# xuyongzhi/Automatic-As-built-Reconstruction

Measured on AMD Instinct MI355X. Metric: scenes/sec (fwd+bwd), higher is better.
Workload: dtype f32

## Files before the change

automatic-as-built-reconstruction_amd/csrc/common.h:

```cpp
#pragma once
#include <hip/hip_runtime.h>
#include <stdint.h>
#include <stdio.h>
#include <atomic>
#include "../../include/aabr_hip.h"
#include "conv_tiles.h"

namespace aabr {

void set_error(const char *fmt, ...);

typedef float f32x4 __attribute__((ext_vector_type(4)));
typedef unsigned int u32x4 __attribute__((ext_vector_type(4)));
typedef __bf16 bf16x8 __attribute__((ext_vector_type(8)));

#define AABR_KNOB_LIST(X)                                                                                            \
  X(CONV_WLDS) X(CONV_SMALL) X(CONV_NBW) X(CONV_WPB) X(WIDE_ROWS) X(CONV_WIDE) X(WIDE_NBUF) X(CONV_WIDE_BF16)         \
  X(VOXEL_MEAN) X(WIDE_NCB) X(BN_SMALL) X(WIDE_PRIO) X(PLAN_SIDE_BATCH) X(PLAN_SIDE_PRIO) X(SMALL_WPB) X(SMALL_MAX)   \
  X(WIDE_SPLIT) X(SPLIT_TARGET) X(SPLIT_NBUF) X(SPLIT_MIN_ITEMS) X(CONV_NARROW) X(DW_FULL) X(DW_FULL_MIN) X(DW_FULL_WGS) X(DW_VEC) X(SPLIT_ROWS) X(GEOM_JOBS)      \
  X(CONV_SINGLE) X(SINGLE_ROWS) X(SINGLE_CHUNK) X(SINGLE_BWD_STATS) X(PLAN_TAIL)
#define AABR_KNOB_ENUM(n) K_##n,
enum Knob { AABR_KNOB_LIST(AABR_KNOB_ENUM) K_COUNT };
#undef AABR_KNOB_ENUM
int knob(Knob k);

#define AABR_CHECK_ARG_AS(fn, cond, msg)                            \
  do {                                                              \
    if (!(cond)) { aabr::set_error("%s: %s", fn, msg); return AABR_EINVAL; } \
  } while (0)
#define AABR_CHECK_ARG(cond, msg) AABR_CHECK_ARG_AS(__func__, cond, msg)

#define AABR_CHECK_LAUNCH()                                                   \
  do {                                                                        \
    hipError_t e__ = hipGetLastError();                                       \
    if (e__ != hipSuccess) {                                                  \
      aabr::set_error("%s: HIP error %s", __func__, hipGetErrorString(e__));  \
      return AABR_ELAUNCH;                                                    \
    }                                                                         \
  } while (0)

#define AABR_CHECK_HIP(call)                                                  \
  do {                                                                        \
    hipError_t e__ = (call);                                                  \
    if (e__ != hipSuccess) {                                                  \
      aabr::set_error("%s: HIP error %s", __func__, hipGetErrorString(e__));  \
      return AABR_ELAUNCH;                                                    \
    }                                                                         \
  } while (0)

struct DynLdsOnce {
  std::atomic<uint64_t> done{0};
};
inline hipError_t dyn_lds_once(DynLdsOnce &o, const void *kernel, int bytes) {
  int dev = 0;
  hipError_t e = hipGetDevice(&dev);
  if (e != hipSuccess) return e;
  const uint64_t bit = dev < 64 ? 1ull << dev : 0ull;
  if (o.done.load(std::memory_order_acquire) & bit) return hipSuccess;
  e = hipFuncSetAttribute(kernel, hipFuncAttributeMaxDynamicSharedMemorySize, bytes);
  if (e == hipSuccess) o.done.fetch_or(bit, std::memory_order_release);
  return e;
}

constexpr uint64_t kEmptyKey = 0xFFFFFFFFFFFFFFFFull;
constexpr int kMaxCoord = 65534;

__host__ __device__ inline uint64_t pack_key(int b, int x, int y, int z) {
  return ((uint64_t)(uint32_t)(b & 0xffff) << 48) | ((uint64_t)(uint32_t)((x + 1) & 0xffff) << 32) |
         ((uint64_t)(uint32_t)((y + 1) & 0xffff) << 16) | (uint64_t)(uint32_t)((z + 1) & 0xffff);
}
__host__ __device__ inline bool coord_in_range(int v) { return v >= -1 && v <= kMaxCoord; }

__host__ __device__ inline uint64_t mix64(uint64_t k) {
  k ^= k >> 33; k *= 0xff51afd7ed558ccdull; k ^= k >> 33;
  k *= 0xc4ceb9fe1a85ec53ull; k ^= k >> 33;
  return k;
}

struct __align__(16) GridEnt {
  unsigned long long key;
  uint32_t first;
  int32_t val;
};
static_assert(sizeof(GridEnt) == 16, "GridEnt is 16 bytes");

constexpr uint32_t kGridBlock = 4096;
__device__ inline uint64_t grid_next(uint64_t h, uint64_t mask, uint32_t t) {
  const uint64_t bm = mask < (uint64_t)(kGridBlock - 1) ? mask : (uint64_t)(kGridBlock - 1);
  return t < bm ? ((h & ~bm) | ((h + 1) & bm)) : (((t == bm ? (h | bm) : h) + 1) & mask);
}

__device__ inline int grid_find(const GridEnt *__restrict__ g, uint64_t mask, uint64_t key) {
  uint64_t h = mix64(key) & mask;
  for (uint32_t t = 0;; ++t) {
    const uint4 e = *reinterpret_cast<const uint4 *>(g + h);
    const uint64_t k = (uint64_t)e.x | ((uint64_t)e.y << 32);
    if (k == key) return (int)e.w;
    if (k == kEmptyKey) return -1;
    h = grid_next(h, mask, t);
  }
}

__device__ inline uint32_t grid_insert(GridEnt *g, uint64_t mask, uint64_t key) {
  uint64_t h = mix64(key) & mask;
  for (uint32_t t = 0;; ++t) {
    unsigned long long prev = atomicCAS(&g[h].key, (unsigned long long)kEmptyKey, (unsigned long long)key);
    if (prev == kEmptyKey || prev == key) return (uint32_t)h;
    h = grid_next(h, mask, t);
  }
}

constexpr int kStreamJobsMax = 48;
struct StreamJob {
  const int32_t *table;
  const int32_t *counts;
  int32_t *words;
  int64_t V;
  int32_t vol, T;
};
struct StreamJobs {
  StreamJob j[kStreamJobsMax];
  uint32_t first[kStreamJobsMax + 1];
  int n;
};
__device__ inline int stream_job_of(const StreamJobs &js, unsigned b) {
  int j = 0;
  while (j + 1 < js.n && b >= js.first[j + 1]) ++j;
  return j;
}
int launch_wide_blocks_jobs(const StreamJob *jobs, int n, hipStream_t st);
int launch_tile_blocks_jobs(const StreamJob *jobs, int n, hipStream_t st);
int launch_offset_pairs_jobs(const StreamJob *jobs, int n, hipStream_t st);
constexpr int kSampleJobsMax = 32;
struct SampleJob {
  const int32_t *sc, *meta;
  int32_t *out;
  int64_t V_max;
  int32_t max_samples;
};
int launch_sample_offsets_jobs(const SampleJob *jobs, int n, hipStream_t st);

inline bool is_pow2(int64_t v) { return v > 0 && (v & (v - 1)) == 0; }

}
```

automatic-as-built-reconstruction_amd/csrc/conv_wide.hip:

```cpp
#include "common.h"
#include "conv_wide_tiles.h"
#include <stdlib.h>

namespace aabr {


extern thread_local const char *g_last_variant;

constexpr int kNB = 4;

__global__ __launch_bounds__(256) void k_build_tileT(const StreamJobs js) {
  const int job = stream_job_of(js, blockIdx.x);
  const int32_t *__restrict__ table = js.j[job].table;
  int32_t *__restrict__ words = js.j[job].words;
  const int64_t V = js.j[job].V;
  const int vol = js.j[job].vol, T = js.j[job].T;
  const int kT = T;
  const int NWV = (T + 63) / 64;
  __shared__ int s_cnt[4][kMaxVol];
  __shared__ int s_base[kMaxVol + 1];
  __shared__ int s_tot[kMaxVol];
  __shared__ int s_first[kMaxVol];
  const int wave = threadIdx.x >> 6, lane = threadIdx.x & 63;
  const int64_t ntiles = (V + T - 1) / T, tile = blockIdx.x - js.first[job];
  const int maxb = (T / 16) * vol;
  int32_t *pre = words + tile * (vol + 1);
  int32_t *ent = words + ntiles * (vol + 1) + tile * (int64_t)maxb * 16;
  const int64_t row = tile * kT + threadIdx.x;
  const bool valid = (int)threadIdx.x < T && row < V;
  for (int k = 0; k < vol; ++k) {
    const int t = valid ? table[(int64_t)k * V + row] : -1;
    const unsigned long long m = __ballot(t >= 0);
    if (lane == 0) s_cnt[wave][k] = __popcll(m);
  }
  __syncthreads();
  if (threadIdx.x == 0) {
    int b = 0;
    for (int k = 0; k < vol; ++k) {
      int tot = 0;
      for (int w = 0; w < NWV; ++w) tot += s_cnt[w][k];
      s_tot[k] = tot;
      s_base[k] = b;
      b += (tot + 15) >> 4;
    }
    s_base[vol] = b;
  }
  __syncthreads();
  if ((int)threadIdx.x <= vol) pre[threadIdx.x] = s_base[threadIdx.x];
  for (int k = 0; k < vol; ++k) {
    const int t = valid ? table[(int64_t)k * V + row] : -1;
    const unsigned long long m = __ballot(t >= 0);
    if (t >= 0) {
      int rank = __popcll(m & ((1ull << lane) - 1ull));
      for (int w = 0; w < wave; ++w) rank += s_cnt[w][k];
      const int e = (t << 8) | (int)threadIdx.x;
      ent[s_base[k] * 16 + rank] = e;
      if (rank == 0) s_first[k] = e;
    }
  }
  __syncthreads();
  for (int k = 0; k < vol; ++k) {
    const int tot = s_tot[k];
    if (tot == 0) continue;
    const int pad = ((tot + 15) & ~15) - tot;
    if ((int)threadIdx.x < pad) ent[s_base[k] * 16 + tot + threadIdx.x] = s_first[k] | (int)0x80000000;
  }
}

__device__ inline float bcf_(unsigned int v) { return __builtin_bit_cast(float, v); }


typedef __bf16 bf16x8w __attribute__((ext_vector_type(8)));
typedef __bf16 bf16x4w __attribute__((ext_vector_type(4)));
typedef unsigned int u32x2 __attribute__((ext_vector_type(2)));

struct BnBwdStats {
  const float *x, *mean, *invstd, *weight, *bias;
  float leak;
  const float *out;
};

template <int KG, int DBG, int NBUF, bool BF = false, int NCB = 1, int NSET = 2>
__global__ __launch_bounds__(256, NBUF == 2 ? 2 : 3) void k_conv_cs(const float *__restrict__ in, int ci, int64_t in_bytes,
                                                    float *__restrict__ out, int co, int64_t V_out,
                                                    const int32_t *__restrict__ words, int64_t words_bytes, int vol,
                                                    int wflip, const float *__restrict__ Wp, int64_t wp_bytes,
                                                    const float *__restrict__ bias, int kT2,
                                                    const float *__restrict__ res, double *__restrict__ stats,
                                                    BnBwdStats bn) {
  constexpr int NW = 4;
  constexpr int NT = 64 * NW;
  constexpr int LPR = NT / 32;
  constexpr int RG = KG * 8;
  constexpr int RF = KG * 32;
  constexpr int SWZ = (RG >= 16 && (RG & 15) == 0) ? 15 : 7;
  constexpr int STAGE = 2 * 16 * RF;
  constexpr bool BFM = BF;
  constexpr int NP = 1;
  constexpr int NGL = KG * 8 / LPR;
  extern __shared__ __align__(16) float smem[];
  float *Ct = smem;
  constexpr int WS = 16 * NW * NCB;
  float *St = smem + (kT2 + 1) * WS;
  const int wave = __builtin_amdgcn_readfirstlane(threadIdx.x >> 6), lane = threadIdx.x & 63;
  const int g = lane >> 4, c16 = lane & 15;
  const int pr = wave * (64 / LPR) + lane / LPR, seg = lane % LPR;
  const int nkc = BFM ? ci >> 6 : ci >> 5, nnb = co >> 4;
  const int nparts = (wflip >> 8) & 0xff;
  int64_t tile;
  int nb0, part = 0;
  {
    const unsigned ny = gridDim.y, total = gridDim.x * ny;
    const unsigned lin = blockIdx.y * gridDim.x + blockIdx.x;
    const unsigned per = total >> 3, rem = total & 7u, x = lin & 7u;
    const unsigned wi = x * per + (x < rem ? x : rem) + (lin >> 3);
    tile = wi / ny;
    unsigned sp = wi % ny;
    if (nparts > 1) { part = (int)(sp % (unsigned)nparts); sp /= (unsigned)nparts; }
    nb0 = (int)sp * (NW * NCB);
  }
  const int k_lo = nparts > 1 ? part * vol / nparts : 0;
  const int kend = nparts > 1 ? (part + 1) * vol / nparts : vol;
  const int64_t row0 = tile * kT2;
  const int64_t ntiles = (V_out + kT2 - 1) / kT2;
  const int maxb = (kT2 / 16) * vol;
  const int vpre = lane <= vol ? words[tile * (vol + 1) + lane] : 0;
  {
    f32x4 z = {0.f, 0.f, 0.f, 0.f};
    f32x4 *c4 = reinterpret_cast<f32x4 *>(Ct);
    for (int i = threadIdx.x; i < (kT2 + 1) * WS / 4; i += NT) c4[i] = z;
  }
  const __amdgpu_buffer_rsrc_t rin =
      __builtin_amdgcn_make_buffer_rsrc(const_cast<float *>(in), 0, (int)in_bytes, 0x00020000);
  const __amdgpu_buffer_rsrc_t rwords =
      __builtin_amdgcn_make_buffer_rsrc(const_cast<int32_t *>(words), 0, (int)words_bytes, 0x00020000);
  const __amdgpu_buffer_rsrc_t rw =
      __builtin_amdgcn_make_buffer_rsrc(const_cast<float *>(Wp), 0, (int)wp_bytes, 0x00020000);
  const unsigned ebase = (unsigned)((ntiles * (vol + 1) + tile * (int64_t)maxb * 16) * 4);
  const unsigned rowbytes = (unsigned)ci * (BF ? 2u : 4u);
  const unsigned lane32 = (unsigned)lane * 32u;
  auto pre_of = [&](int k) { return __builtin_amdgcn_readlane(vpre, k); };
  auto next_offset = [&](int k) {
    ++k;
    while (k < kend && pre_of(k + 1) == pre_of(k)) ++k;
    return k;
  };
  struct WReg { u32x4 w0[NP][NCB][KG], w1[NP][NCB][KG]; };
  struct GReg { u32x4 v[NGL]; };
  struct Ent { int eg, ea, eb, hb; };
  const int ngroups = (nkc + KG - 1) / KG;
  const int nblk_all = pre_of(vol);
  auto load_w = [&](WReg &w, int k, int kg) {
    const int kW = (wflip & 1) ? vol - 1 - k : k;
#pragma unroll
    for (int cb = 0; cb < NCB; ++cb)
#pragma unroll
      for (int c = 0; c < KG; ++c) {
        const int kc = kg * KG + c;
        if (BFM) {
          const unsigned so = (unsigned)((((int64_t)kW * (2 * nkc) + 2 * kc) * nnb + nb0 + wave * NCB + cb) * 1024);
#pragma unroll
          for (int pl = 0; pl < NP; ++pl) {
            const unsigned po = so + (unsigned)pl * (unsigned)(wp_bytes / NP);
            w.w0[pl][cb][c] = __builtin_amdgcn_raw_buffer_load_b128(rw, (unsigned)lane * 16u, po, 0);
            w.w1[pl][cb][c] = __builtin_amdgcn_raw_buffer_load_b128(rw, (unsigned)lane * 16u, po + (unsigned)nnb * 1024u, 0);
          }
        } else {
          const unsigned so = (unsigned)((((int64_t)kW * nkc + kc) * nnb + nb0 + wave * NCB + cb) * 2048);
          w.w0[0][cb][c] = __builtin_amdgcn_raw_buffer_load_b128(rw, lane32, so, 0);
          w.w1[0][cb][c] = __builtin_amdgcn_raw_buffer_load_b128(rw, lane32 + 16u, so, 0);
        }
      }
  };
  auto load_ent = [&](int bb, int kk) {
    Ent e;
    const bool hasB = bb + 1 < pre_of(kk + 1);
    const unsigned bA = (unsigned)bb * 64u, bB = (unsigned)(hasB ? bb + 1 : bb) * 64u;
    e.ea = (int)__builtin_amdgcn_raw_buffer_load_b32(rwords, (unsigned)c16 * 4u, ebase + bA, 0);
    e.eb = (int)__builtin_amdgcn_raw_buffer_load_b32(rwords, (unsigned)c16 * 4u, ebase + bB, 0);
    e.eg = (int)__builtin_amdgcn_raw_buffer_load_b32(rwords, (unsigned)(pr & 15) * 4u, ebase + (pr < 16 ? bA : bB), 0);
    if (!hasB) e.eb |= (int)0x80000000;
    e.hb = hasB ? 1 : 0;
    return e;
  };
  auto gather = [&](GReg &q, int eg, int kg) {
    const unsigned va = (((unsigned)eg & 0x7fffffffu) >> 8) * rowbytes + (unsigned)seg * 16u;
#pragma unroll
    for (int i = 0; i < NGL; ++i) {
      const unsigned so = (unsigned)(kg * NGL + i) * (unsigned)(LPR * 16);
      if (DBG & 2) q.v[i] = (u32x4){(unsigned)eg, 0u, 0u, 0u};
      else q.v[i] = __builtin_amdgcn_raw_buffer_load_b128(rin, va, so, 0);
    }
  };
  auto stage_store = [&](const GReg &q, int buf) {
    float *rowp = St + (NBUF == 2 ? buf : 0) * (NP * STAGE) + pr * RF;
#pragma unroll
    for (int i = 0; i < NGL; ++i)
      *reinterpret_cast<u32x4 *>(rowp + (((seg + LPR * i) ^ (pr & SWZ)) << 2)) = q.v[i];
  };
  auto accumulate2 = [&](int ea, const f32x4 (&accA)[NCB], int eb, const f32x4 (&accB)[NCB]) {
    const int ra = ea >= 0 ? (ea & 255) : kT2, rb = eb >= 0 ? (eb & 255) : kT2;
#pragma unroll
    for (int cb = 0; cb < NCB; ++cb) {
      f32x4 *da = reinterpret_cast<f32x4 *>(Ct + ra * WS + ((((wave * NCB + cb) * 4 + g) ^ (ra & 15)) << 2));
      f32x4 *db = reinterpret_cast<f32x4 *>(Ct + rb * WS + ((((wave * NCB + cb) * 4 + g) ^ (rb & 15)) << 2));
      const f32x4 va = *da, vb = *db;
      *da = va + accA[cb];
      *db = vb + accB[cb];
    }
  };
  struct Pos { int b, k; };
  auto adv = [&](Pos q) {
    if (q.k >= kend) return q;
    const int kend = pre_of(q.k + 1);
    q.b += 2;
    if (q.b >= kend) { q.b = kend; q.k = next_offset(q.k); }
    return q;
  };
  auto wg_barrier = [&]() {
    asm volatile("s_waitcnt lgkmcnt(0)\n\ts_barrier" ::: "memory");
  };
  int par = 0;
  long long dbg_t[5] = {0, 0, 0, 0, 0};
  for (int kg = 0; kg < ngroups; ++kg) {
    Pos pp[NSET + 2];
    pp[0].k = next_offset(k_lo - 1);
    if (pp[0].k >= kend) break;
    pp[0].b = pre_of(pp[0].k);
#pragma unroll
    for (int i = 1; i < NSET + 2; ++i) pp[i] = adv(pp[i - 1]);
    auto ent_of = [&](const Pos &q) { const bool v = q.k < kend; return load_ent(v ? q.b : pp[0].b, v ? q.k : pp[0].k); };
    Ent ee[NSET + 2];
#pragma unroll
    for (int i = 0; i <= NSET; ++i) ee[i] = ent_of(pp[i]);
    ee[NSET + 1] = ee[0];
    GReg gq[NSET];
    gather(gq[0], ee[0].eg, kg);
    __syncthreads();
    par = 0;
    int gs = 0;
    stage_store(gq[0], par);
#pragma unroll
    for (int i = 1; i < NSET; ++i) gather(gq[i], ee[i].eg, kg);
    __syncthreads();
    auto step = [&](const WReg &w, GReg &g_issue, GReg &g_store) __attribute__((always_inline)) {
      long long t0 = 0, t1 = 0, t2 = 0, t3 = 0, t4 = 0;
      if (DBG & 4) t0 = __builtin_amdgcn_s_memtime();
      gather(g_issue, ee[NSET].eg, kg);
      ee[NSET + 1] = ent_of(pp[NSET + 1]);
      const Ent e0 = ee[0];
      __builtin_amdgcn_sched_barrier(0);
      if (DBG & 4) { t1 = __builtin_amdgcn_s_memtime(); __builtin_amdgcn_sched_barrier(0); }

      {
        const float *sa = St + (NBUF == 2 ? par : 0) * STAGE + c16 * RF;
        const float *sb = sa + 16 * RF;
        f32x4 accA[NCB], accB[NCB];
#pragma unroll
        for (int cb = 0; cb < NCB; ++cb) { accA[cb] = (f32x4){0.f, 0.f, 0.f, 0.f}; accB[cb] = accA[cb]; }
        if (wflip & 2) __builtin_amdgcn_s_setprio(3);
        {
        u32x4 a0[KG], a1[KG], b0[KG], b1[KG];
#pragma unroll
        for (int c = 0; c < KG; ++c) {
          const int q0 = ((c * 8 + (BF ? g : g * 2)) ^ (c16 & SWZ)) << 2,
                    q1 = ((c * 8 + (BF ? 4 + g : g * 2 + 1)) ^ (c16 & SWZ)) << 2;
          a0[c] = *reinterpret_cast<const u32x4 *>(sa + q0);
          b0[c] = *reinterpret_cast<const u32x4 *>(sb + q0);
          a1[c] = *reinterpret_cast<const u32x4 *>(sa + q1);
          b1[c] = *reinterpret_cast<const u32x4 *>(sb + q1);
        }
        if (DBG & 1) {
#pragma unroll
          for (int c = 0; c < KG; ++c) {
            accA[0][0] += bcf_(a0[c][0]) + bcf_(a1[c][0]) + bcf_(w.w0[0][0][c][0]) + bcf_(w.w1[0][0][c][0]);
            accB[0][0] += bcf_(b0[c][0]) + bcf_(b1[c][0]);
          }
        } else if (BF) {
#pragma unroll
          for (int cb = 0; cb < NCB; ++cb)
#pragma unroll
            for (int c = 0; c < KG; ++c) {
              accA[cb] = __builtin_amdgcn_mfma_f32_16x16x32_bf16(__builtin_bit_cast(bf16x8w, w.w0[0][cb][c]),
                                                                 __builtin_bit_cast(bf16x8w, a0[c]), accA[cb], 0, 0, 0);
              accA[cb] = __builtin_amdgcn_mfma_f32_16x16x32_bf16(__builtin_bit_cast(bf16x8w, w.w1[0][cb][c]),
                                                                 __builtin_bit_cast(bf16x8w, a1[c]), accA[cb], 0, 0, 0);
            }
          if (e0.hb) {
#pragma unroll
            for (int cb = 0; cb < NCB; ++cb)
#pragma unroll
              for (int c = 0; c < KG; ++c) {
                accB[cb] = __builtin_amdgcn_mfma_f32_16x16x32_bf16(__builtin_bit_cast(bf16x8w, w.w0[0][cb][c]),
                                                                   __builtin_bit_cast(bf16x8w, b0[c]), accB[cb], 0, 0, 0);
                accB[cb] = __builtin_amdgcn_mfma_f32_16x16x32_bf16(__builtin_bit_cast(bf16x8w, w.w1[0][cb][c]),
                                                                   __builtin_bit_cast(bf16x8w, b1[c]), accB[cb], 0, 0, 0);
              }
          }
        } else {
#pragma unroll
          for (int cb = 0; cb < NCB; ++cb)
#pragma unroll
            for (int c = 0; c < KG; ++c) {
#pragma unroll
              for (int t = 0; t < 4; ++t)
                accA[cb] = __builtin_amdgcn_mfma_f32_16x16x4f32(bcf_(w.w0[0][cb][c][t]), bcf_(a0[c][t]), accA[cb], 0, 0, 0);
#pragma unroll
              for (int t = 0; t < 4; ++t)
                accA[cb] = __builtin_amdgcn_mfma_f32_16x16x4f32(bcf_(w.w1[0][cb][c][t]), bcf_(a1[c][t]), accA[cb], 0, 0, 0);
            }
          if (e0.hb) {
#pragma unroll
            for (int cb = 0; cb < NCB; ++cb)
#pragma unroll
              for (int c = 0; c < KG; ++c) {
#pragma unroll
                for (int t = 0; t < 4; ++t)
                  accB[cb] = __builtin_amdgcn_mfma_f32_16x16x4f32(bcf_(w.w0[0][cb][c][t]), bcf_(b0[c][t]), accB[cb], 0, 0, 0);
#pragma unroll
                for (int t = 0; t < 4; ++t)
                  accB[cb] = __builtin_amdgcn_mfma_f32_16x16x4f32(bcf_(w.w1[0][cb][c][t]), bcf_(b1[c][t]), accB[cb], 0, 0, 0);
              }
          }
        }
        }
        if (DBG & 4) { __builtin_amdgcn_sched_barrier(0); asm volatile("s_nop 0" ::"v"(accA[0]), "v"(accB[0])); t2 = __builtin_amdgcn_s_memtime(); __builtin_amdgcn_sched_barrier(0); }
        if (wflip & 2) __builtin_amdgcn_s_setprio(0);
        {
          accumulate2(e0.ea, accA, e0.eb, accB);
        }
      }
      {
        if (NBUF == 1) wg_barrier();
        if (pp[1].k < kend) stage_store(g_store, par ^ 1);
      }
      if (DBG & 4) { asm volatile("s_waitcnt lgkmcnt(0)" ::: "memory"); t3 = __builtin_amdgcn_s_memtime(); }
      wg_barrier();
      if (DBG & 4) {
        t4 = __builtin_amdgcn_s_memtime();
        dbg_t[0] += t1 - t0; dbg_t[1] += t2 - t1; dbg_t[2] += t3 - t2; dbg_t[3] += t4 - t3; dbg_t[4] += 1;
      }
      par ^= 1;
#pragma unroll
      for (int i = 0; i < NSET + 1; ++i) { pp[i] = pp[i + 1]; ee[i] = ee[i + 1]; }
      pp[NSET + 1] = adv(pp[NSET + 1]);
    };
    auto step2 = [&](const WReg &w) __attribute__((always_inline)) {
      if (NSET == 2) {
        if (gs == 0) step(w, gq[0], gq[1]);
        else step(w, gq[1], gq[0]);
      } else {
        if (gs == 0) step(w, gq[0], gq[1 % NSET]);
        else if (gs == 1) step(w, gq[1 % NSET], gq[2 % NSET]);
        else if (gs == 2) step(w, gq[2 % NSET], gq[3 % NSET]);
        else step(w, gq[3 % NSET], gq[0]);
      }
      gs = gs + 1 == NSET ? 0 : gs + 1;
    };
    WReg wA;
    int k = pp[0].k;
    load_w(wA, k, kg);
    WReg wB;
    for (;;) {
      int kn = next_offset(k);
      if (kn < kend) load_w(wB, kn, kg);
      while (pp[0].k == k) step2(wA);
      if (kn >= kend) break;
      k = kn;
      kn = next_offset(k);
      if (kn < kend) load_w(wA, kn, kg);
      while (pp[0].k == k) step2(wB);
      if (kn >= kend) break;
      k = kn;
    }
  }
  if (DBG & 4) {
    if (lane == 0) {
      long long *d = reinterpret_cast<long long *>(const_cast<float *>(bias)) +
                     (((int64_t)blockIdx.y * gridDim.x + blockIdx.x) * 4 + wave) * 5;
      for (int q = 0; q < 5; ++q) d[q] = dbg_t[q];
    }
    bias = nullptr;
  }
  __syncthreads();
  const int nrows = (int)((V_out - row0) < kT2 ? (V_out - row0) : kT2);
  constexpr int QW = 4 * NW * NCB;
  if (nparts > 1) {
    float *po = out + (int64_t)part * V_out * co;
    for (int i = threadIdx.x; i < nrows * QW; i += NT) {
      const int r = i / QW, q = i % QW;
      *reinterpret_cast<f32x4 *>(po + (row0 + r) * co + nb0 * 16 + q * 4) =
          *reinterpret_cast<const f32x4 *>(Ct + r * WS + ((q ^ (r & 15)) << 2));
    }
    return;
  }
  double sa[4] = {0.0, 0.0, 0.0, 0.0}, sb[4] = {0.0, 0.0, 0.0, 0.0};
  float bmu[4] = {0.f, 0.f, 0.f, 0.f}, bwc[4] = {0.f, 0.f, 0.f, 0.f}, bbc[4] = {0.f, 0.f, 0.f, 0.f};
  if (stats && bn.x) {
    const int p0 = nb0 * 16 + (threadIdx.x % QW) * 4;
#pragma unroll
    for (int j = 0; j < 4; ++j) {
      bmu[j] = bn.mean[p0 + j];
      if (!BF) {
        bwc[j] = bn.invstd[p0 + j] * (bn.weight ? bn.weight[p0 + j] : 1.0f);
        bbc[j] = -bmu[j] * bwc[j] + (bn.bias ? bn.bias[p0 + j] : 0.0f);
      }
    }
  }
#pragma unroll 4
  for (int i = threadIdx.x; i < nrows * QW; i += NT) {
    const int r = i / QW, q = i % QW;
    f32x4 v = *reinterpret_cast<const f32x4 *>(Ct + r * WS + ((q ^ (r & 15)) << 2));
    if (bias) {
      const float *bb = bias + nb0 * 16 + q * 4;
      v[0] += bb[0]; v[1] += bb[1]; v[2] += bb[2]; v[3] += bb[3];
    }
    if (res) {
      if (BF) {
        const bf16x4w rr = *reinterpret_cast<const bf16x4w *>(reinterpret_cast<const __bf16 *>(res) + (row0 + r) * co +
                                                              nb0 * 16 + q * 4);
#pragma unroll
        for (int j = 0; j < 4; ++j) v[j] = (float)(__bf16)v[j] + (float)rr[j];
      } else {
        const f32x4 rr = *reinterpret_cast<const f32x4 *>(res + (row0 + r) * co + nb0 * 16 + q * 4);
        v[0] += rr[0]; v[1] += rr[1]; v[2] += rr[2]; v[3] += rr[3];
      }
    }
    if (BF) {
      bf16x4w o = {(__bf16)v[0], (__bf16)v[1], (__bf16)v[2], (__bf16)v[3]};
      *reinterpret_cast<bf16x4w *>(reinterpret_cast<__bf16 *>(out) + (row0 + r) * co + nb0 * 16 + q * 4) = o;
      if (stats) { v[0] = (float)o[0]; v[1] = (float)o[1]; v[2] = (float)o[2]; v[3] = (float)o[3]; }
    } else {
      *reinterpret_cast<f32x4 *>(out + (row0 + r) * co + nb0 * 16 + q * 4) = v;
    }
    if (stats) {
      if (BF && bn.x) {
        const int64_t at = (row0 + r) * co + nb0 * 16 + q * 4;
        const bf16x4w xv = *reinterpret_cast<const bf16x4w *>(reinterpret_cast<const __bf16 *>(bn.x) + at);
        const bf16x4w ov = *reinterpret_cast<const bf16x4w *>(reinterpret_cast<const __bf16 *>(bn.out) + at);
#pragma unroll
        for (int j = 0; j < 4; ++j) {
          const float d = ((float)ov[j] > 0.0f) ? v[j] : v[j] * bn.leak;
          sa[j] += (double)d;
          sb[j] += (double)((float)xv[j] - bmu[j]) * (double)d;
        }
      } else if (bn.x) {
        const f32x4 xv = *reinterpret_cast<const f32x4 *>(bn.x + (row0 + r) * co + nb0 * 16 + q * 4);
#pragma unroll
        for (int j = 0; j < 4; ++j) {
          const float o = xv[j] * bwc[j] + bbc[j];
          const float d = (o > 0.0f) ? v[j] : v[j] * bn.leak;
          sa[j] += (double)d;
          sb[j] += (double)(xv[j] - bmu[j]) * (double)d;
        }
      } else {
#pragma unroll
        for (int j = 0; j < 4; ++j) { sa[j] += (double)v[j]; sb[j] += (double)v[j] * (double)v[j]; }
      }
    }
  }
  if (stats) {
    __syncthreads();
    double *red = reinterpret_cast<double *>(smem);
#pragma unroll
    for (int j = 0; j < 4; ++j) { red[threadIdx.x * 8 + j] = sa[j]; red[threadIdx.x * 8 + 4 + j] = sb[j]; }
    __syncthreads();
    if (threadIdx.x < 16 * NW * NCB) {
      const int q = threadIdx.x >> 2, j = threadIdx.x & 3;
      double a = 0.0, b = 0.0;
#pragma unroll
      for (int t = 0; t < NT / QW; ++t) { a += red[(t * QW + q) * 8 + j]; b += red[(t * QW + q) * 8 + 4 + j]; }
      stats[(tile * 2 + 0) * co + nb0 * 16 + threadIdx.x] = a;
      stats[(tile * 2 + 1) * co + nb0 * 16 + threadIdx.x] = b;
    }
  }
}

}
using namespace aabr;

extern "C" int64_t aabr_wide_blocks_words(int64_t V, int vol, int tile_rows) { return wide_words(V, vol, tile_rows); }

extern "C" int aabr_build_wide_blocks(const int32_t *table, int64_t V, int vol, int tile_rows, int32_t *blocks,
                                      void *stream_) {
  AABR_CHECK_ARG(V >= 0 && vol > 0 && vol <= kMaxVol, "bad sizes (vol <= 63)");
  AABR_CHECK_ARG(tile_rows >= 16 && tile_rows <= kMaxTileRows && (tile_rows & 15) == 0, "tile_rows: multiple of 16, <= 240");
  if (V == 0) return AABR_OK;
  AABR_CHECK_ARG(table && blocks, "null pointer");
  const StreamJob job{table, nullptr, blocks, V, vol, tile_rows};
  return launch_wide_blocks_jobs(&job, 1, (hipStream_t)stream_);
}

int aabr::launch_wide_blocks_jobs(const StreamJob *jobs, int n, hipStream_t st) {
  for (int nwv = 1; nwv <= 4; ++nwv) {
    StreamJobs js;
    js.n = 0;
    uint64_t blocks = 0;
    auto flush = [&]() -> int {
      if (js.n == 0 || blocks == 0) { js.n = 0; blocks = 0; return AABR_OK; }
      js.first[js.n] = (uint32_t)blocks;
      hipLaunchKernelGGL(k_build_tileT, dim3((unsigned)blocks), dim3(64 * nwv), 0, st, js);
      js.n = 0;
      blocks = 0;
      return AABR_OK;
    };
    for (int j = 0; j < n; ++j) {
      if ((jobs[j].T + 63) / 64 != nwv) continue;
      const uint64_t b = (uint64_t)((jobs[j].V + jobs[j].T - 1) / jobs[j].T);
      if (js.n == kStreamJobsMax || blocks + b >= (1ull << 31)) flush();
      AABR_CHECK_ARG(b < (1ull << 31), "too many tiles in one rule book");
      js.j[js.n] = jobs[j];
      js.first[js.n] = (uint32_t)blocks;
      blocks += b;
      ++js.n;
    }
    flush();
  }
  AABR_CHECK_LAUNCH();
  return AABR_OK;
}

static WideKnobs wide_knobs() {
  return {knob(K_WIDE_ROWS), knob(K_CONV_WIDE), knob(K_CONV_WIDE_BF16), knob(K_WIDE_SPLIT), knob(K_SPLIT_ROWS),
          knob(K_SPLIT_MIN_ITEMS), knob(K_SPLIT_TARGET), knob(K_WIDE_NBUF), knob(K_SPLIT_NBUF), knob(K_WIDE_NCB),
          knob(K_WIDE_PRIO)};
}

extern "C" int aabr_conv_wide_tile_rows(int n_in, int n_out, int64_t rows_in, int64_t V_out, int vol) {
  return wide_tile_rows(kWideF32, n_in, n_out, rows_in, V_out, vol, wide_knobs());
}
extern "C" int aabr_conv_wide_tile_rows_bf16(int n_in, int n_out, int64_t rows_in, int64_t V_out, int vol) {
  return wide_tile_rows(kWideBf16, n_in, n_out, rows_in, V_out, vol, wide_knobs());
}
extern "C" int aabr_conv_wide_split(int n_in, int n_out, int64_t rows_in, int64_t V_out, int vol) {
  return wide_split(kWideF32, n_in, n_out, rows_in, V_out, vol, wide_knobs());
}
extern "C" int aabr_conv_wide_split_bf16(int n_in, int n_out, int64_t rows_in, int64_t V_out, int vol) {
  return wide_split(kWideBf16, n_in, n_out, rows_in, V_out, vol, wide_knobs());
}

extern "C" int64_t aabr_conv_wide_stats_doubles(int64_t V_out, int tile_rows, int n_out) {
  if (V_out <= 0 || tile_rows <= 0 || n_out <= 0) return 0;
  return ((V_out + tile_rows - 1) / tile_rows) * 2 * n_out;
}

extern "C" int64_t aabr_conv_wide_split_scratch_floats(int64_t V_out, int n_out, int parts) {
  return V_out > 0 && n_out > 0 && parts > 0 ? (int64_t)parts * V_out * n_out : 0;
}

namespace aabr {
template <bool BF>
__global__ __launch_bounds__(256) void k_split_reduce(const float *__restrict__ parts, int nparts, int64_t n4, int co4,
                                                      const float *__restrict__ bias, const float *__restrict__ res,
                                                      void *__restrict__ out) {
  const int64_t i = (int64_t)blockIdx.x * 256 + threadIdx.x;
  if (i >= n4) return;
  f32x4 v = reinterpret_cast<const f32x4 *>(parts)[i];
  for (int p = 1; p < nparts; ++p) {
    const f32x4 w = reinterpret_cast<const f32x4 *>(parts)[(int64_t)p * n4 + i];
    v[0] += w[0]; v[1] += w[1]; v[2] += w[2]; v[3] += w[3];
  }
  if (bias) {
    const float *bb = bias + (i % co4) * 4;
    v[0] += bb[0]; v[1] += bb[1]; v[2] += bb[2]; v[3] += bb[3];
  }
  if (res) {
    if (BF) {
      const bf16x4w rr = reinterpret_cast<const bf16x4w *>(res)[i];
#pragma unroll
      for (int j = 0; j < 4; ++j) v[j] = (float)(__bf16)v[j] + (float)rr[j];
    } else {
      const f32x4 rr = reinterpret_cast<const f32x4 *>(res)[i];
      v[0] += rr[0]; v[1] += rr[1]; v[2] += rr[2]; v[3] += rr[3];
    }
  }
  if (BF) {
    bf16x4w o = {(__bf16)v[0], (__bf16)v[1], (__bf16)v[2], (__bf16)v[3]};
    reinterpret_cast<bf16x4w *>(out)[i] = o;
  } else {
    reinterpret_cast<f32x4 *>(out)[i] = v;
  }
}
}

typedef decltype(&k_conv_cs<1, 0, 1>) WideFn;
struct WideInst {
  WideKernel k;
  const char *name, *split_name;
  WideFn fn;
};
static const WideInst kWide[] = {
    {{1, 0, 1, false, 1, false}, "k_conv_cs<1,0,1>", nullptr, k_conv_cs<1, 0, 1>},
    {{1, 0, 2, false, 1, false}, "k_conv_cs<1,0,2>", nullptr, k_conv_cs<1, 0, 2>},
    {{2, 0, 1, false, 1, false}, "k_conv_cs<2,0,1>", "k_conv_cs<2,0,1,split>", k_conv_cs<2, 0, 1>},
    {{2, 0, 2, false, 1, false}, "k_conv_cs<2,0,2>", "k_conv_cs<2,0,2,split>", k_conv_cs<2, 0, 2>},
    {{3, 0, 1, false, 1, false}, "k_conv_cs<3,0,1>", "k_conv_cs<3,0,1,split>", k_conv_cs<3, 0, 1>},
    {{3, 0, 2, false, 1, false}, "k_conv_cs<3,0,2>", "k_conv_cs<3,0,2,split>", k_conv_cs<3, 0, 2>},
    {{4, 0, 1, false, 1, false}, "k_conv_cs<4,0,1>", "k_conv_cs<4,0,1,split>", k_conv_cs<4, 0, 1>},
    {{4, 0, 2, false, 1, false}, "k_conv_cs<4,0,2>", "k_conv_cs<4,0,2,split>", k_conv_cs<4, 0, 2>},
    {{1, 0, 1, true, 1, false}, "k_conv_cs<1,0,1,bf16>", "k_conv_cs<1,0,1,bf16,split>", k_conv_cs<1, 0, 1, true, 1>},
    {{1, 0, 2, true, 1, false}, "k_conv_cs<1,0,2,bf16>", nullptr, k_conv_cs<1, 0, 2, true, 1>},
    {{1, 0, 1, true, 2, false}, "k_conv_cs<1,0,1,bf16,x128>", nullptr, k_conv_cs<1, 0, 1, true, 2>},
    {{1, 0, 2, true, 2, false}, "k_conv_cs<1,0,2,bf16,x128>", nullptr, k_conv_cs<1, 0, 2, true, 2>},
    {{2, 0, 1, true, 1, false}, "k_conv_cs<2,0,1,bf16>", "k_conv_cs<2,0,1,bf16,split>", k_conv_cs<2, 0, 1, true, 1>},
    {{2, 0, 2, true, 1, false}, "k_conv_cs<2,0,2,bf16>", nullptr, k_conv_cs<2, 0, 2, true, 1>},
    {{2, 0, 1, true, 2, false}, "k_conv_cs<2,0,1,bf16,x128>", nullptr, k_conv_cs<2, 0, 1, true, 2>},
    {{2, 0, 2, true, 2, false}, "k_conv_cs<2,0,2,bf16,x128>", nullptr, k_conv_cs<2, 0, 2, true, 2>},
    {{3, 0, 1, true, 1, false}, "k_conv_cs<3,0,1,bf16>", "k_conv_cs<3,0,1,bf16,split>", k_conv_cs<3, 0, 1, true, 1>},
    {{3, 0, 2, true, 1, false}, "k_conv_cs<3,0,2,bf16>", nullptr, k_conv_cs<3, 0, 2, true, 1>},
    {{4, 0, 1, true, 1, false}, "k_conv_cs<4,0,1,bf16>", "k_conv_cs<4,0,1,bf16,split>", k_conv_cs<4, 0, 1, true, 1>},
    {{4, 0, 2, true, 1, false}, "k_conv_cs<4,0,2,bf16>", nullptr, k_conv_cs<4, 0, 2, true, 1>},
#ifdef AABR_DEV
    {{4, 1, 1, false, 1, false}, "k_conv_cs<4,1,1>", nullptr, k_conv_cs<4, 1, 1>},
    {{4, 1, 2, false, 1, false}, "k_conv_cs<4,1,2>", nullptr, k_conv_cs<4, 1, 2>},
    {{4, 2, 1, false, 1, false}, "k_conv_cs<4,2,1>", nullptr, k_conv_cs<4, 2, 1>},
    {{4, 2, 2, false, 1, false}, "k_conv_cs<4,2,2>", nullptr, k_conv_cs<4, 2, 2>},
    {{4, 3, 1, false, 1, false}, "k_conv_cs<4,3,1>", nullptr, k_conv_cs<4, 3, 1>},
    {{4, 3, 2, false, 1, false}, "k_conv_cs<4,3,2>", nullptr, k_conv_cs<4, 3, 2>},
    {{4, 4, 1, false, 1, false}, "k_conv_cs<4,4,1>", nullptr, k_conv_cs<4, 4, 1>},
    {{4, 4, 2, false, 1, false}, "k_conv_cs<4,4,2>", nullptr, k_conv_cs<4, 4, 2>},
    {{2, 4, 1, true, 1, false}, "k_conv_cs<2,4,1,bf16>", nullptr, k_conv_cs<2, 4, 1, true, 1>},
    {{2, 4, 1, true, 2, false}, "k_conv_cs<2,4,1,bf16,x128>", nullptr, k_conv_cs<2, 4, 1, true, 2>},
#endif
};
constexpr int kWideCount = sizeof(kWide) / sizeof(kWide[0]);
static DynLdsOnce kWideLds[kWideCount];

struct WideArgs {
  const char *fn;
  int storage;
  const void *in;
  int n_in;
  int64_t rows_in;
  void *out;
  int n_out;
  int64_t V_out;
  const int32_t *blocks;
  int tile_rows, vol;
  const float *bias;
  int flags;
  const void *wpack, *residual;
  double *stats;
  BnBwdStats bn;
  bool split;
  int parts;
  float *scratch;
  void *stream;
};

static int wide_run(const WideArgs &a) {
  hipStream_t st = (hipStream_t)a.stream;
  const WideStorageDesc &s = wide_storage(a.storage);
  const bool bf16 = a.storage == kWideBf16;
  AABR_CHECK_ARG_AS(a.fn, !a.split || (a.parts != 0 && a.scratch && ((uintptr_t)a.scratch & 15) == 0),
                    "2 <= parts <= min(32, vol) and a 16-byte aligned scratch of parts x V_out x n_out floats");
  AABR_CHECK_ARG_AS(a.fn, ((uintptr_t)a.residual & (s.res_align - 1)) == 0,
                    bf16 ? "residual must be 8-byte aligned" : "residual must be 16-byte aligned");
  AABR_CHECK_ARG_AS(a.fn, ((uintptr_t)a.stats & 7) == 0, "statistics need tiles of >= 64 rows");
  WideLaunch t;
  const char *refused = wide_launch(a.storage, a.split ? a.parts : 0, a.n_in, a.n_out, a.rows_in, a.V_out, a.tile_rows,
                                    a.vol, a.flags, a.stats != nullptr, wide_knobs(), t);
  AABR_CHECK_ARG_AS(a.fn, !refused, refused);
  if (a.V_out == 0) return AABR_OK;
  AABR_CHECK_ARG_AS(a.fn, a.in && a.out && a.blocks && a.wpack, "null pointer / empty input");
  AABR_CHECK_ARG_AS(a.fn, (((uintptr_t)a.in | (uintptr_t)a.out | (uintptr_t)a.wpack) & 15) == 0,
                    "feature / weight pointers must be 16-byte aligned");
  WideKernel k = t.k;
  k.split = false;
  const WideInst *e = nullptr;
  for (int i = 0; i < kWideCount && !e; ++i)
    if (kWide[i].k == k) e = &kWide[i];
  AABR_CHECK_ARG_AS(a.fn, e && (!a.split || e->split_name), "no kernel instance for this launch");
  AABR_CHECK_HIP(dyn_lds_once(kWideLds[e - kWide], (const void *)e->fn, 80 * 1024));
  g_last_variant = a.split ? e->split_name : e->name;
  const dim3 grid((unsigned)t.grid_x, (unsigned)t.grid_y);
  const float *in = static_cast<const float *>(a.in), *wp = static_cast<const float *>(a.wpack);
  if (a.split) {
    hipLaunchKernelGGL(e->fn, grid, dim3(256), (size_t)t.lds_bytes, st, in, a.n_in, t.in_bytes, a.scratch, a.n_out, a.V_out,
                       a.blocks, t.words_bytes, a.vol, t.wflip, wp, t.wp_bytes, (const float *)nullptr, a.tile_rows,
                       (const float *)nullptr, (double *)nullptr, BnBwdStats{});
    const int64_t n4 = a.V_out * a.n_out / 4;
    const dim3 rgrid((unsigned)((n4 + 255) / 256));
    const float *res = static_cast<const float *>(a.residual);
    if (bf16)
      hipLaunchKernelGGL((k_split_reduce<true>), rgrid, dim3(256), 0, st, a.scratch, a.parts, n4, a.n_out / 4, a.bias, res, a.out);
    else
      hipLaunchKernelGGL((k_split_reduce<false>), rgrid, dim3(256), 0, st, a.scratch, a.parts, n4, a.n_out / 4, a.bias, res, a.out);
  } else {
    hipLaunchKernelGGL(e->fn, grid, dim3(256), (size_t)t.lds_bytes, st, in, a.n_in, t.in_bytes, static_cast<float *>(a.out),
                       a.n_out, a.V_out, a.blocks, t.words_bytes, a.vol, t.wflip, wp, t.wp_bytes, a.bias, a.tile_rows,
                       static_cast<const float *>(a.residual), a.stats, a.bn);
  }
  AABR_CHECK_LAUNCH();
  return AABR_OK;
}

extern "C" int aabr_conv_forward_wide_stats(const float *in_feats, int n_in, int64_t rows_in, float *out_feats,
                                            int n_out, int64_t V_out, const int32_t *blocks, int tile_rows, int vol,
                                            const float *bias, int flags, const float *wpack, const float *residual,
                                            double *stats, void *stream_) {
  return wide_run({__func__, kWideF32, in_feats, n_in, rows_in, out_feats, n_out, V_out, blocks, tile_rows, vol, bias, flags,
                   wpack, residual, stats, BnBwdStats{}, false, 0, nullptr, stream_});
}

extern "C" int aabr_conv_forward_wide_res(const float *in_feats, int n_in, int64_t rows_in, float *out_feats,
                                          int n_out, int64_t V_out, const int32_t *blocks, int tile_rows, int vol,
                                          const float *bias, int flags, const float *wpack, const float *residual,
                                          void *stream_) {
  return wide_run({__func__, kWideF32, in_feats, n_in, rows_in, out_feats, n_out, V_out, blocks, tile_rows, vol, bias, flags,
                   wpack, residual, nullptr, BnBwdStats{}, false, 0, nullptr, stream_});
}

extern "C" int aabr_conv_forward_wide(const float *in_feats, int n_in, int64_t rows_in, float *out_feats, int n_out,
                                      int64_t V_out, const int32_t *blocks, int tile_rows, int vol, const float *bias,
                                      int flags, const float *wpack, void *stream_) {
  return wide_run({__func__, kWideF32, in_feats, n_in, rows_in, out_feats, n_out, V_out, blocks, tile_rows, vol, bias, flags,
                   wpack, nullptr, nullptr, BnBwdStats{}, false, 0, nullptr, stream_});
}

extern "C" int aabr_conv_forward_wide_bwd_stats(const float *in_feats, int n_in, int64_t rows_in, float *out_feats,
                                                int n_out, int64_t V_out, const int32_t *blocks, int tile_rows, int vol,
                                                const float *bias, int flags, const float *wpack, const float *residual,
                                                double *stats, const float *bn_in, const float *save_mean,
                                                const float *save_invstd, const float *bn_weight, const float *bn_bias,
                                                float leakiness, void *stream_) {
  AABR_CHECK_ARG(stats && bn_in && save_mean && save_invstd, "null pointer");
  AABR_CHECK_ARG(leakiness >= 0.0f, "the activation sign is recomputed from the BatchNorm input: leakiness >= 0");
  AABR_CHECK_ARG(((uintptr_t)bn_in & 15) == 0, "the BatchNorm input must be 16-byte aligned");
  return wide_run({__func__, kWideF32, in_feats, n_in, rows_in, out_feats, n_out, V_out, blocks, tile_rows, vol, bias, flags,
                   wpack, residual, stats, BnBwdStats{bn_in, save_mean, save_invstd, bn_weight, bn_bias, leakiness}, false, 0,
                   nullptr, stream_});
}

extern "C" int aabr_conv_forward_wide_split(const float *in_feats, int n_in, int64_t rows_in, float *out_feats, int n_out,
                                            int64_t V_out, const int32_t *blocks, int tile_rows, int vol,
                                            const float *bias, int flags, const float *wpack, const float *residual,
                                            int parts, float *scratch, void *stream_) {
  return wide_run({__func__, kWideF32, in_feats, n_in, rows_in, out_feats, n_out, V_out, blocks, tile_rows, vol, bias, flags,
                   wpack, residual, nullptr, BnBwdStats{}, true, parts, scratch, stream_});
}

static BnBwdStats bf16_bwd_stats(const uint16_t *bn_in, const uint16_t *bn_out, const float *save_mean, float leakiness) {
  return BnBwdStats{reinterpret_cast<const float *>(bn_in), save_mean, nullptr, nullptr, nullptr, leakiness,
                    reinterpret_cast<const float *>(bn_out)};
}

extern "C" int aabr_conv_forward_wide_bf16_stats(const uint16_t *in_feats, int n_in, int64_t rows_in,
                                                 uint16_t *out_feats, int n_out, int64_t V_out, const int32_t *blocks,
                                                 int tile_rows, int vol, const float *bias, int flags,
                                                 const uint16_t *wpack, double *stats, void *stream_) {
  return wide_run({__func__, kWideBf16, in_feats, n_in, rows_in, out_feats, n_out, V_out, blocks, tile_rows, vol, bias, flags,
                   wpack, nullptr, stats, BnBwdStats{}, false, 0, nullptr, stream_});
}

extern "C" int aabr_conv_forward_wide_bf16(const uint16_t *in_feats, int n_in, int64_t rows_in, uint16_t *out_feats,
                                           int n_out, int64_t V_out, const int32_t *blocks, int tile_rows, int vol,
                                           const float *bias, int flags, const uint16_t *wpack, void *stream_) {
  return wide_run({__func__, kWideBf16, in_feats, n_in, rows_in, out_feats, n_out, V_out, blocks, tile_rows, vol, bias, flags,
                   wpack, nullptr, nullptr, BnBwdStats{}, false, 0, nullptr, stream_});
}

extern "C" int aabr_conv_forward_wide_bf16_res(const uint16_t *in_feats, int n_in, int64_t rows_in, uint16_t *out_feats,
                                               int n_out, int64_t V_out, const int32_t *blocks, int tile_rows, int vol,
                                               const float *bias, int flags, const uint16_t *wpack,
                                               const uint16_t *residual, double *stats, const uint16_t *bn_in,
                                               const uint16_t *bn_out, const float *save_mean, float leakiness,
                                               void *stream_) {
  if (bn_in) {
    AABR_CHECK_ARG(stats && bn_out && save_mean, "null pointer");
    AABR_CHECK_ARG((((uintptr_t)bn_in | (uintptr_t)bn_out) & 7) == 0, "the BatchNorm's input / output must be 8-byte aligned");
  }
  return wide_run({__func__, kWideBf16, in_feats, n_in, rows_in, out_feats, n_out, V_out, blocks, tile_rows, vol, bias, flags,
                   wpack, residual, stats, bn_in ? bf16_bwd_stats(bn_in, bn_out, save_mean, leakiness) : BnBwdStats{}, false,
                   0, nullptr, stream_});
}

extern "C" int aabr_conv_forward_wide_bf16_bwd_stats(const uint16_t *in_feats, int n_in, int64_t rows_in,
                                                     uint16_t *out_feats, int n_out, int64_t V_out,
                                                     const int32_t *blocks, int tile_rows, int vol, const float *bias,
                                                     int flags, const uint16_t *wpack, double *stats,
                                                     const uint16_t *bn_in, const uint16_t *bn_out,
                                                     const float *save_mean, float leakiness, void *stream_) {
  AABR_CHECK_ARG(stats && bn_in && bn_out && save_mean, "null pointer");
  AABR_CHECK_ARG((((uintptr_t)bn_in | (uintptr_t)bn_out) & 7) == 0, "the BatchNorm's input / output must be 8-byte aligned");
  return wide_run({__func__, kWideBf16, in_feats, n_in, rows_in, out_feats, n_out, V_out, blocks, tile_rows, vol, bias, flags,
                   wpack, nullptr, stats, bf16_bwd_stats(bn_in, bn_out, save_mean, leakiness), false, 0, nullptr, stream_});
}

extern "C" int aabr_conv_forward_wide_split_bf16_res(const uint16_t *in_feats, int n_in, int64_t rows_in,
                                                     uint16_t *out_feats, int n_out, int64_t V_out, const int32_t *blocks,
                                                     int tile_rows, int vol, const float *bias, int flags,
                                                     const uint16_t *wpack, int parts, float *scratch,
                                                     const uint16_t *residual, void *stream_) {
  return wide_run({__func__, kWideBf16, in_feats, n_in, rows_in, out_feats, n_out, V_out, blocks, tile_rows, vol, bias, flags,
                   wpack, residual, nullptr, BnBwdStats{}, true, parts, scratch, stream_});
}

extern "C" int aabr_conv_forward_wide_split_bf16(const uint16_t *in_feats, int n_in, int64_t rows_in, uint16_t *out_feats,
                                                 int n_out, int64_t V_out, const int32_t *blocks, int tile_rows, int vol,
                                                 const float *bias, int flags, const uint16_t *wpack, int parts,
                                                 float *scratch, void *stream_) {
  return wide_run({__func__, kWideBf16, in_feats, n_in, rows_in, out_feats, n_out, V_out, blocks, tile_rows, vol, bias, flags,
                   wpack, nullptr, nullptr, BnBwdStats{}, true, parts, scratch, stream_});
}
```

Before: 354.0.

## Add cross-offset pipelined path to wide fp32 conv kernel for small KG

Adds an XO template variant of the wide sparse-conv kernel for fp32 with KG <= 2. It walks the tile's block list two blocks at a time, so consecutive blocks belonging to different kernel offsets are processed in one pipelined step with separate weight registers, rather than iterating group by group per offset. This aims to cut per-offset loop overhead and keep the MFMA and gather pipeline full when offsets contain few blocks. The variant raises the launch-bounds occupancy hint to 4 waves and is selected by a new WIDE_XOFF knob for non-split launches, at the cost of more register pressure and duplicated kernel instances.

```diff
diff --git a/automatic-as-built-reconstruction_amd/csrc/common.h b/automatic-as-built-reconstruction_amd/csrc/common.h
--- a/automatic-as-built-reconstruction_amd/csrc/common.h
+++ b/automatic-as-built-reconstruction_amd/csrc/common.h
@@ -18,7 +18,7 @@
   X(CONV_WLDS) X(CONV_SMALL) X(CONV_NBW) X(CONV_WPB) X(WIDE_ROWS) X(CONV_WIDE) X(WIDE_NBUF) X(CONV_WIDE_BF16)         \
   X(VOXEL_MEAN) X(WIDE_NCB) X(BN_SMALL) X(WIDE_PRIO) X(PLAN_SIDE_BATCH) X(PLAN_SIDE_PRIO) X(SMALL_WPB) X(SMALL_MAX)   \
   X(WIDE_SPLIT) X(SPLIT_TARGET) X(SPLIT_NBUF) X(SPLIT_MIN_ITEMS) X(CONV_NARROW) X(DW_FULL) X(DW_FULL_MIN) X(DW_FULL_WGS) X(DW_VEC) X(SPLIT_ROWS) X(GEOM_JOBS)      \
-  X(CONV_SINGLE) X(SINGLE_ROWS) X(SINGLE_CHUNK) X(SINGLE_BWD_STATS) X(PLAN_TAIL)
+  X(CONV_SINGLE) X(SINGLE_ROWS) X(SINGLE_CHUNK) X(SINGLE_BWD_STATS) X(PLAN_TAIL) X(WIDE_XOFF)
 #define AABR_KNOB_ENUM(n) K_##n,
 enum Knob { AABR_KNOB_LIST(AABR_KNOB_ENUM) K_COUNT };
 #undef AABR_KNOB_ENUM
diff --git a/automatic-as-built-reconstruction_amd/csrc/conv_wide.hip b/automatic-as-built-reconstruction_amd/csrc/conv_wide.hip
--- a/automatic-as-built-reconstruction_amd/csrc/conv_wide.hip
+++ b/automatic-as-built-reconstruction_amd/csrc/conv_wide.hip
@@ -1,6 +1,7 @@
 #include "common.h"
 #include "conv_wide_tiles.h"
 #include <stdlib.h>
+#include <type_traits>
 
 namespace aabr {
 
@@ -80,8 +81,8 @@
   const float *out;
 };
 
-template <int KG, int DBG, int NBUF, bool BF = false, int NCB = 1, int NSET = 2>
-__global__ __launch_bounds__(256, NBUF == 2 ? 2 : 3) void k_conv_cs(const float *__restrict__ in, int ci, int64_t in_bytes,
+template <int KG, int DBG, int NBUF, bool BF = false, int NCB = 1, int NSET = 2, bool XO = false>
+__global__ __launch_bounds__(256, XO ? 4 : NBUF == 2 ? 2 : 3) void k_conv_cs(const float *__restrict__ in, int ci, int64_t in_bytes,
                                                     float *__restrict__ out, int co, int64_t V_out,
                                                     const int32_t *__restrict__ words, int64_t words_bytes, int vol,
                                                     int wflip, const float *__restrict__ Wp, int64_t wp_bytes,
@@ -222,6 +223,128 @@
   };
   int par = 0;
   long long dbg_t[5] = {0, 0, 0, 0, 0};
+  if constexpr (XO) {
+    static_assert(!BF && NCB == 1 && NSET == 2 && DBG == 0 && KG <= 2, "the cross-offset step exists for fp32, KG <= 2");
+    const int nblk = nblk_all;
+    struct XPos { int b, ka, kb; };
+    auto off_from = [&](int k, int b) { while (pre_of(k + 1) <= b) ++k; return k; };
+    auto xadv = [&](XPos q) {
+      if (q.b >= nblk) return q;
+      q.b += 2;
+      if (q.b >= nblk) { q.b = nblk; return q; }
+      q.ka = off_from(q.kb, q.b);
+      q.kb = q.b + 1 < nblk ? off_from(q.ka, q.b + 1) : q.ka;
+      return q;
+    };
+    struct XEnt { int w, hb; };
+    XPos pp[NSET + 2];
+    XEnt ee[NSET + 2];
+    auto xent_of = [&](const XPos &q) {
+      const int b = q.b < nblk ? q.b : pp[0].b;
+      XEnt e;
+      e.w = (int)__builtin_amdgcn_raw_buffer_load_b32(rwords, (unsigned)(lane & 31) * 4u, ebase + (unsigned)b * 64u, 0);
+      e.hb = b + 1 < nblk ? 1 : 0;
+      return e;
+    };
+    auto eg_of = [&](const XEnt &e) { return __builtin_amdgcn_ds_bpermute((e.hb ? pr : (pr & 15)) << 2, e.w); };
+    auto accumulate1 = [&](int e, const f32x4 &acc) {
+      const int r = e >= 0 ? (e & 255) : kT2;
+      f32x4 *d = reinterpret_cast<f32x4 *>(Ct + r * WS + (((wave * 4 + g) ^ (r & 15)) << 2));
+      *d = *d + acc;
+    };
+    if (nblk > 0) {
+      pp[0].b = 0;
+      pp[0].ka = off_from(0, 0);
+      pp[0].kb = 1 < nblk ? off_from(pp[0].ka, 1) : pp[0].ka;
+#pragma unroll
+      for (int i = 1; i < NSET + 2; ++i) pp[i] = xadv(pp[i - 1]);
+#pragma unroll
+      for (int i = 0; i <= NSET; ++i) ee[i] = xent_of(pp[i]);
+      ee[NSET + 1] = ee[0];
+      GReg gq[NSET];
+      gather(gq[0], eg_of(ee[0]), 0);
+      __syncthreads();
+      stage_store(gq[0], 0);
+      gather(gq[1], eg_of(ee[1]), 0);
+      __syncthreads();
+      auto kA_next = [&]() { return pp[1].b < nblk ? pp[1].ka : pp[0].ka; };
+      auto kB_next = [&]() { return pp[1].b < nblk ? pp[1].kb : pp[0].kb; };
+      WReg WA, WB;
+      load_w(WA, pp[0].ka, 0);
+      load_w(WB, pp[0].kb, 0);
+      auto step = [&](GReg &g_issue, GReg &g_store) __attribute__((always_inline)) {
+        gather(g_issue, eg_of(ee[NSET]), 0);
+        ee[NSET + 1] = xent_of(pp[NSET + 1]);
+        const XEnt e0 = ee[0];
+        const int ea = __builtin_amdgcn_ds_bpermute(c16 << 2, e0.w);
+        const int eb = __builtin_amdgcn_ds_bpermute((e0.hb ? 16 + c16 : c16) << 2, e0.w) | (e0.hb ? 0 : (int)0x80000000);
+        __builtin_amdgcn_sched_barrier(0);
+        const float *sa_ = St + (NBUF == 2 ? par : 0) * STAGE + c16 * RF;
+        const float *sb_ = sa_ + 16 * RF;
+        f32x4 accA = {0.f, 0.f, 0.f, 0.f}, accB = accA;
+        if (wflip & 2) __builtin_amdgcn_s_setprio(3);
+        {
+          u32x4 a0[KG], a1[KG], b0[KG], b1[KG];
+#pragma unroll
+          for (int c = 0; c < KG; ++c) {
+            const int q0 = ((c * 8 + g * 2) ^ (c16 & SWZ)) << 2, q1 = ((c * 8 + g * 2 + 1) ^ (c16 & SWZ)) << 2;
+            a0[c] = *reinterpret_cast<const u32x4 *>(sa_ + q0);
+            b0[c] = *reinterpret_cast<const u32x4 *>(sb_ + q0);
+            a1[c] = *reinterpret_cast<const u32x4 *>(sa_ + q1);
+            b1[c] = *reinterpret_cast<const u32x4 *>(sb_ + q1);
+          }
+#pragma unroll
+          for (int c = 0; c < KG; ++c) {
+#pragma unroll
+            for (int t = 0; t < 4; ++t)
+              accA = __builtin_amdgcn_mfma_f32_16x16x4f32(bcf_(WA.w0[0][0][c][t]), bcf_(a0[c][t]), accA, 0, 0, 0);
+#pragma unroll
+            for (int t = 0; t < 4; ++t)
+              accA = __builtin_amdgcn_mfma_f32_16x16x4f32(bcf_(WA.w1[0][0][c][t]), bcf_(a1[c][t]), accA, 0, 0, 0);
+          }
+          __builtin_amdgcn_sched_barrier(0);
+          load_w(WA, kA_next(), 0);
+          __builtin_amdgcn_sched_barrier(0);
+          if (e0.hb) {
+#pragma unroll
+            for (int c = 0; c < KG; ++c) {
+#pragma unroll
+              for (int t = 0; t < 4; ++t)
+                accB = __builtin_amdgcn_mfma_f32_16x16x4f32(bcf_(WB.w0[0][0][c][t]), bcf_(b0[c][t]), accB, 0, 0, 0);
+#pragma unroll
+              for (int t = 0; t < 4; ++t)
+                accB = __builtin_amdgcn_mfma_f32_16x16x4f32(bcf_(WB.w1[0][0][c][t]), bcf_(b1[c][t]), accB, 0, 0, 0);
+            }
+          }
+          __builtin_amdgcn_sched_barrier(0);
+          load_w(WB, kB_next(), 0);
+          __builtin_amdgcn_sched_barrier(0);
+        }
+        if (wflip & 2) __builtin_amdgcn_s_setprio(0);
+        if (pp[0].kb != pp[0].ka) {
+          accumulate1(ea, accA);
+          accumulate1(eb, accB);
+        } else {
+          const f32x4 aA[1] = {accA}, aB[1] = {accB};
+          accumulate2(ea, aA, eb, aB);
+        }
+        if (NBUF == 1) wg_barrier();
+        if (pp[1].b < nblk) stage_store(g_store, par ^ 1);
+        wg_barrier();
+        par ^= 1;
+#pragma unroll
+        for (int i = 0; i < NSET + 1; ++i) { pp[i] = pp[i + 1]; ee[i] = ee[i + 1]; }
+        pp[NSET + 1] = xadv(pp[NSET + 1]);
+      };
+      for (;;) {
+        step(gq[0], gq[1]);
+        if (pp[0].b >= nblk) break;
+        step(gq[1], gq[0]);
+        if (pp[0].b >= nblk) break;
+      }
+    }
+  }
+  if constexpr (!XO)
   for (int kg = 0; kg < ngroups; ++kg) {
     Pos pp[NSET + 2];
     pp[0].k = next_offset(k_lo - 1);
@@ -588,12 +711,17 @@
   WideKernel k;
   const char *name, *split_name;
   WideFn fn;
+  WideFn fn_xoff = nullptr;
 };
 static const WideInst kWide[] = {
-    {{1, 0, 1, false, 1, false}, "k_conv_cs<1,0,1>", nullptr, k_conv_cs<1, 0, 1>},
-    {{1, 0, 2, false, 1, false}, "k_conv_cs<1,0,2>", nullptr, k_conv_cs<1, 0, 2>},
-    {{2, 0, 1, false, 1, false}, "k_conv_cs<2,0,1>", "k_conv_cs<2,0,1,split>", k_conv_cs<2, 0, 1>},
-    {{2, 0, 2, false, 1, false}, "k_conv_cs<2,0,2>", "k_conv_cs<2,0,2,split>", k_conv_cs<2, 0, 2>},
+    {{1, 0, 1, false, 1, false}, "k_conv_cs<1,0,1>", nullptr, k_conv_cs<1, 0, 1>,
+     k_conv_cs<1, 0, 1, false, 1, 2, true>},
+    {{1, 0, 2, false, 1, false}, "k_conv_cs<1,0,2>", nullptr, k_conv_cs<1, 0, 2>,
+     k_conv_cs<1, 0, 2, false, 1, 2, true>},
+    {{2, 0, 1, false, 1, false}, "k_conv_cs<2,0,1>", "k_conv_cs<2,0,1,split>", k_conv_cs<2, 0, 1>,
+     k_conv_cs<2, 0, 1, false, 1, 2, true>},
+    {{2, 0, 2, false, 1, false}, "k_conv_cs<2,0,2>", "k_conv_cs<2,0,2,split>", k_conv_cs<2, 0, 2>,
+     k_conv_cs<2, 0, 2, false, 1, 2, true>},
     {{3, 0, 1, false, 1, false}, "k_conv_cs<3,0,1>", "k_conv_cs<3,0,1,split>", k_conv_cs<3, 0, 1>},
     {{3, 0, 2, false, 1, false}, "k_conv_cs<3,0,2>", "k_conv_cs<3,0,2,split>", k_conv_cs<3, 0, 2>},
     {{4, 0, 1, false, 1, false}, "k_conv_cs<4,0,1>", "k_conv_cs<4,0,1,split>", k_conv_cs<4, 0, 1>},
@@ -624,7 +752,7 @@
 #endif
 };
 constexpr int kWideCount = sizeof(kWide) / sizeof(kWide[0]);
-static DynLdsOnce kWideLds[kWideCount];
+static DynLdsOnce kWideLds[kWideCount], kWideLdsX[kWideCount];
 
 struct WideArgs {
   const char *fn;
@@ -671,7 +799,9 @@
   for (int i = 0; i < kWideCount && !e; ++i)
     if (kWide[i].k == k) e = &kWide[i];
   AABR_CHECK_ARG_AS(a.fn, e && (!a.split || e->split_name), "no kernel instance for this launch");
-  AABR_CHECK_HIP(dyn_lds_once(kWideLds[e - kWide], (const void *)e->fn, 80 * 1024));
+  const bool xoff = !a.split && e->fn_xoff && knob(K_WIDE_XOFF) != 0;
+  const WideFn fn = xoff ? e->fn_xoff : e->fn;
+  AABR_CHECK_HIP(dyn_lds_once(xoff ? kWideLdsX[e - kWide] : kWideLds[e - kWide], (const void *)fn, 80 * 1024));
   g_last_variant = a.split ? e->split_name : e->name;
   const dim3 grid((unsigned)t.grid_x, (unsigned)t.grid_y);
   const float *in = static_cast<const float *>(a.in), *wp = static_cast<const float *>(a.wpack);
@@ -687,7 +817,7 @@
     else
       hipLaunchKernelGGL((k_split_reduce<false>), rgrid, dim3(256), 0, st, a.scratch, a.parts, n4, a.n_out / 4, a.bias, res, a.out);
   } else {
-    hipLaunchKernelGGL(e->fn, grid, dim3(256), (size_t)t.lds_bytes, st, in, a.n_in, t.in_bytes, static_cast<float *>(a.out),
+    hipLaunchKernelGGL(fn, grid, dim3(256), (size_t)t.lds_bytes, st, in, a.n_in, t.in_bytes, static_cast<float *>(a.out),
                        a.n_out, a.V_out, a.blocks, t.words_bytes, a.vol, t.wflip, wp, t.wp_bytes, a.bias, a.tile_rows,
                        static_cast<const float *>(a.residual), a.stats, a.bn);
   }
```

After: 359.6, median of 6. 1.6% higher.
